# aipixel/GPS-Gaussian

Measured on NVIDIA H100. Metric: novel_views_per_sec_1024sq_500kgauss, higher is better.
Workload: dtype f32

## Files before the change

### gps-gaussian_b200/csrc/raster_render.cu

```cuda
#include "gpsg_internal.cuh"
#include "sm90_ptx.cuh"

namespace gpsg {

using namespace sm90;

struct f2p { float a, b; };
__device__ __forceinline__ f2p pk2(float lo, float hi) { return {lo, hi}; }
__device__ __forceinline__ void upk2(f2p v, float& lo, float& hi) { lo = v.a; hi = v.b; }
__device__ __forceinline__ f2p sub2(f2p x, f2p y) { return {__fsub_rn(x.a, y.a), __fsub_rn(x.b, y.b)}; }
__device__ __forceinline__ f2p mul2(f2p x, f2p y) { return {__fmul_rn(x.a, y.a), __fmul_rn(x.b, y.b)}; }
__device__ __forceinline__ f2p fma2(f2p x, f2p y, f2p z) { return {__fmaf_rn(x.a, y.a, z.a), __fmaf_rn(x.b, y.b, z.b)}; }

constexpr int kFwdWarps = 2;
constexpr int kFwdCTAsPerTile = 8 / kFwdWarps;
constexpr int kFwdQ = 32;
static_assert(kFwdWarps == 1 || kFwdWarps == 2 || kFwdWarps == 4, "a CTA holds 1, 2 or 4 of a tile's 8 blocks");

template <bool AUX>
struct FwdQueue {
    float4 A[2][kFwdQ], B[2][kFwdQ], C[2][kFwdQ];
    uint32_t pos[2][kFwdQ];
    float z[2][AUX ? kFwdQ : 1];
};

struct FwdPixel {
    float T = 1.0f, C0 = 0.0f, C1 = 0.0f, C2 = 0.0f, D = 0.0f;
    uint32_t last = 0;
    bool done;
};

template <bool AUX>
__device__ __forceinline__ void fwd_eval_pair(const float4& a0, const float4& a1, const float4& b0, const float4& b1,
                                              const float4& c0, const float4& c1, uint2 pos, float2 z, f2p pixfx2, f2p pixfy2,
                                              FwdPixel& px) {
    const f2p dx2 = sub2(pk2(a0.x, a1.x), pixfx2), dy2 = sub2(pk2(a0.y, a1.y), pixfy2);
    const f2p t2 = fma2(pk2(b0.x, b1.x), dx2, mul2(pk2(b0.y, b1.y), dy2));
    const f2p p2 = fma2(mul2(pk2(b0.z, b1.z), dy2), dy2, mul2(t2, dx2));
    float pA, pB;
    upk2(p2, pA, pB);
    float aA, aB;
    upk2(mul2(pk2(b0.w, b1.w), pk2(ex2_approx(pA), ex2_approx(pB))), aA, aB);
#pragma unroll
    for (int u = 0; u < 2; ++u) {
        const float p = u ? pB : pA;
        const float alpha = fminf(0.99f, u ? aB : aA);
        const bool valid = !px.done && !(p > 0.0f) && !(alpha < 1.0f / 255.0f);
        const float test_T = px.T * (1.0f - alpha);
        const bool stop = valid && (test_T < 0.0001f);
        const bool upd = valid && !stop;
        px.done = px.done || stop;
        const float w = upd ? alpha * px.T : 0.0f;
        const float4& c = u ? c1 : c0;
        px.C0 = fmaf(c.x, w, px.C0);
        px.C1 = fmaf(c.y, w, px.C1);
        px.C2 = fmaf(c.z, w, px.C2);
        if constexpr (AUX) px.D = fmaf(u ? z.y : z.x, w, px.D);
        px.T = upd ? test_T : px.T;
        px.last = upd ? (u ? pos.y : pos.x) : px.last;
    }
}

template <bool AUX>
__global__ void __launch_bounds__(kFwdWarps * 32, 32 / kFwdWarps) render_forward_kernel(const __grid_constant__ Camera cam,
                                                                            const float4* __restrict__ slabA,
                                                                            const float4* __restrict__ slabB,
                                                                            const float4* __restrict__ slabC,
                                                                            const uint32_t* __restrict__ blk_list,
                                                                            const uint2* __restrict__ ranges, const uint32_t* __restrict__ tile_order,
                                                                            const uint32_t* __restrict__ blk_count,
                                                                            const uint32_t* __restrict__ status,
                                                                            float* __restrict__ final_T,
                                                                            uint32_t* __restrict__ n_contrib,
                                                                            float* __restrict__ out_color,
                                                                            const float* __restrict__ depths,
                                                                            float* __restrict__ out_depth,
                                                                            float* __restrict__ out_alpha) {
    __shared__ FwdQueue<AUX> queues[kFwdWarps];
    const int lane = threadIdx.x & 31, warp = threadIdx.x >> 5;
    const int tile = (int)tile_order[blockIdx.x / kFwdCTAsPerTile];
    const int blk = (int)(blockIdx.x % kFwdCTAsPerTile) * kFwdWarps + warp;
    const int tile_y = tile / cam.grid_x, tile_x = tile - tile_y * cam.grid_x;
    int bx0, by0;
    fwd_block_origin(tile_x, tile_y, blk, bx0, by0);
    const int px = bx0 + (lane & 7), py = by0 + (lane >> 3);
    const bool inside = px < cam.W && py < cam.H;
    const uint2 range = status[2] ? make_uint2(0u, 0u) : ranges[tile];
    const uint32_t n = range.y - range.x;
    const int cnt = n ? (int)blk_count[8 * tile + blk] : 0;

    FwdPixel pix;
    pix.done = !inside;
    if (cnt > 0 && !__all_sync(0xffffffffu, pix.done)) {
        FwdQueue<AUX>& q = queues[warp];
        const uint32_t* __restrict__ list = blk_list + 8 * (size_t)range.x + (size_t)blk * n;
        const float4* __restrict__ tA = slabA + range.x;
        const float4* __restrict__ tB = slabB + range.x;
        const float4* __restrict__ tC = slabC + range.x;
        const f2p pixfx2 = pk2((float)px, (float)px), pixfy2 = pk2((float)py, (float)py);
        auto fetch = [&](int c, int buf, uint32_t p) {
            const int m = min(kFwdQ, cnt - c);
            if (lane < m) {
                cp_async16(&q.A[buf][lane], tA + p);
                cp_async16(&q.B[buf][lane], tB + p);
                cp_async16(&q.C[buf][lane], tC + p);
                q.pos[buf][lane] = p + 1u;
            } else if (lane == m && (m & 1)) {
                const float4 zero = make_float4(0.f, 0.f, 0.f, 0.f);
                q.A[buf][lane] = zero; q.B[buf][lane] = zero; q.C[buf][lane] = zero;
                q.pos[buf][lane] = 0u;
                if constexpr (AUX) q.z[buf][lane] = 0.f;
            }
        };
        auto fetch_z = [&](int c, int buf, uint32_t id) {
            if (lane < cnt - c) cp_async4(&q.z[buf][lane], depths + id);
        };
        uint32_t p = lane < cnt ? list[lane] : 0u;
        uint32_t id = 0u;
        fetch(0, 0, p);
        cp_async_commit();
        if constexpr (AUX) {
            if (lane < cnt) id = __float_as_uint(tC[p].w);
            fetch_z(0, 0, id);
            cp_async_commit();
        }
        p = lane + kFwdQ < cnt ? list[lane + kFwdQ] : 0u;
        for (int c = 0, buf = 0; c < cnt; c += kFwdQ, buf ^= 1) {
            const bool more = c + kFwdQ < cnt;
            if (more) {
                fetch(c + kFwdQ, buf ^ 1, p);
                if constexpr (AUX) { if (lane < cnt - c - kFwdQ) id = __float_as_uint(tC[p].w); }
                if (c + 2 * kFwdQ + lane < cnt) p = list[c + 2 * kFwdQ + lane];
            }
            cp_async_commit();
            cp_async_wait1();
            __syncwarp();
            const int m = min(kFwdQ, cnt - c);
#pragma unroll 2
            for (int i = 0; i < m; i += 2) {
                float2 z = make_float2(0.f, 0.f);
                if constexpr (AUX) z = *reinterpret_cast<const float2*>(&q.z[buf][i]);
                fwd_eval_pair<AUX>(q.A[buf][i], q.A[buf][i + 1], q.B[buf][i], q.B[buf][i + 1], q.C[buf][i], q.C[buf][i + 1],
                                   *reinterpret_cast<const uint2*>(&q.pos[buf][i]), z, pixfx2, pixfy2, pix);
            }
            __syncwarp();
            if (__all_sync(0xffffffffu, pix.done)) break;
            if constexpr (AUX) {
                if (more) fetch_z(c + kFwdQ, buf ^ 1, id);
                cp_async_commit();
            }
        }
        cp_async_wait_all();
    }

    if (inside) {
        const size_t HW = (size_t)cam.W * cam.H;
        const size_t pid = (size_t)py * cam.W + px;
        final_T[pid] = pix.T;
        n_contrib[pid] = pix.last;
        out_color[pid] = fmaf(pix.T, cam.bg[0], pix.C0);
        out_color[HW + pid] = fmaf(pix.T, cam.bg[1], pix.C1);
        out_color[2 * HW + pid] = fmaf(pix.T, cam.bg[2], pix.C2);
        if constexpr (AUX) {
            out_depth[pid] = pix.D;
            out_alpha[pid] = 1.0f - pix.T;
        }
    }
}

int launch_render_forward(const Camera& cam, BinningState b, ImageState im, float* out_color, const float* depths,
                          float* out_depth, float* out_alpha, cudaStream_t stream) {
    const unsigned grid = (unsigned)kFwdCTAsPerTile * (unsigned)(cam.grid_x * cam.grid_y);
    if (out_depth)
        render_forward_kernel<true><<<grid, kFwdWarps * 32, 0, stream>>>(
            cam, b.slabA, b.slabB, b.slabC, b.blk_list, im.ranges, im.tile_order, im.blk_count, im.totals, im.final_T,
            im.n_contrib, out_color, depths, out_depth, out_alpha);
    else
        render_forward_kernel<false><<<grid, kFwdWarps * 32, 0, stream>>>(
            cam, b.slabA, b.slabB, b.slabC, b.blk_list, im.ranges, im.tile_order, im.blk_count, im.totals, im.final_T,
            im.n_contrib, out_color, nullptr, nullptr, nullptr);
    GPSG_LAUNCH_CHECK();
    return GPSG_OK;
}

}
```

### gps-gaussian_b200/csrc/sm90_ptx.cuh

```cuda
#pragma once
#include <stdint.h>

namespace gpsg {
namespace sm90 {

__device__ __forceinline__ uint32_t smem_addr(const void* p) { return (uint32_t)__cvta_generic_to_shared(p); }

__device__ __forceinline__ float tf32(float x) {
    uint32_t r;
    asm("cvt.rna.tf32.f32 %0, %1;" : "=r"(r) : "f"(x));
    return __uint_as_float(r);
}

__device__ __forceinline__ float ex2_approx(float x) {
    float y;
    asm("ex2.approx.ftz.f32 %0, %1;" : "=f"(y) : "f"(x));
    return y;
}

__device__ __forceinline__ float rcp_approx(float x) {
    float y;
    asm("rcp.approx.ftz.f32 %0, %1;" : "=f"(y) : "f"(x));
    return y;
}

__device__ __forceinline__ uint32_t opaque(uint32_t x) {
    uint32_t y;
    asm volatile("mov.u32 %0, %1;" : "=r"(y) : "r"(x));
    return y;
}

__device__ __forceinline__ unsigned long long globaltimer() {
    unsigned long long t;
    asm volatile("mov.u64 %0, %%globaltimer;" : "=l"(t));
    return t;
}

__device__ __forceinline__ uint64_t gmma_desc(uint32_t addr, uint32_t lbo_bytes, uint32_t sbo_bytes) {
    uint64_t d = 0;
    d |= (uint64_t)((addr & 0x3FFFFu) >> 4);
    d |= (uint64_t)((lbo_bytes >> 4) & 0x3FFFu) << 16;
    d |= (uint64_t)((sbo_bytes >> 4) & 0x3FFFu) << 32;
    return d;
}

__device__ __forceinline__ void wgmma_m64n32k8(float (&d)[16], uint64_t a_desc, uint64_t b_desc) {
    asm volatile(
        "{\n\t.reg .pred p;\n\tsetp.ne.b32 p, %18, 0;\n\t"
        "wgmma.mma_async.sync.aligned.m64n32k8.f32.tf32.tf32 "
        "{%0, %1, %2, %3, %4, %5, %6, %7, %8, %9, %10, %11, %12, %13, %14, %15}, %16, %17, p, 1, 1;\n\t}"
        : "+f"(d[0]), "+f"(d[1]), "+f"(d[2]), "+f"(d[3]), "+f"(d[4]), "+f"(d[5]), "+f"(d[6]), "+f"(d[7]), "+f"(d[8]), "+f"(d[9]), "+f"(d[10]), "+f"(d[11]), "+f"(d[12]), "+f"(d[13]), "+f"(d[14]), "+f"(d[15])
        : "l"(a_desc), "l"(b_desc), "n"(1)
        : "memory");
}

__device__ __forceinline__ void wgmma_m64n48k8(float (&d)[24], uint64_t a_desc, uint64_t b_desc) {
    asm volatile(
        "{\n\t.reg .pred p;\n\tsetp.ne.b32 p, %26, 0;\n\t"
        "wgmma.mma_async.sync.aligned.m64n48k8.f32.tf32.tf32 "
        "{%0, %1, %2, %3, %4, %5, %6, %7, %8, %9, %10, %11, %12, %13, %14, %15, %16, %17, %18, %19, %20, %21, %22, %23}, %24, %25, p, 1, 1;\n\t}"
        : "+f"(d[0]), "+f"(d[1]), "+f"(d[2]), "+f"(d[3]), "+f"(d[4]), "+f"(d[5]), "+f"(d[6]), "+f"(d[7]), "+f"(d[8]), "+f"(d[9]), "+f"(d[10]), "+f"(d[11]), "+f"(d[12]), "+f"(d[13]), "+f"(d[14]), "+f"(d[15]), "+f"(d[16]), "+f"(d[17]), "+f"(d[18]), "+f"(d[19]), "+f"(d[20]), "+f"(d[21]), "+f"(d[22]), "+f"(d[23])
        : "l"(a_desc), "l"(b_desc), "n"(1)
        : "memory");
}

__device__ __forceinline__ void wgmma_m64n56k8(float (&d)[28], uint64_t a_desc, uint64_t b_desc) {
    asm volatile(
        "{\n\t.reg .pred p;\n\tsetp.ne.b32 p, %30, 0;\n\t"
        "wgmma.mma_async.sync.aligned.m64n56k8.f32.tf32.tf32 "
        "{%0, %1, %2, %3, %4, %5, %6, %7, %8, %9, %10, %11, %12, %13, %14, %15, %16, %17, %18, %19, %20, %21, %22, %23, %24, %25, %26, %27}, %28, %29, p, 1, 1;\n\t}"
        : "+f"(d[0]), "+f"(d[1]), "+f"(d[2]), "+f"(d[3]), "+f"(d[4]), "+f"(d[5]), "+f"(d[6]), "+f"(d[7]), "+f"(d[8]), "+f"(d[9]), "+f"(d[10]), "+f"(d[11]), "+f"(d[12]), "+f"(d[13]), "+f"(d[14]), "+f"(d[15]), "+f"(d[16]), "+f"(d[17]), "+f"(d[18]), "+f"(d[19]), "+f"(d[20]), "+f"(d[21]), "+f"(d[22]), "+f"(d[23]), "+f"(d[24]), "+f"(d[25]), "+f"(d[26]), "+f"(d[27])
        : "l"(a_desc), "l"(b_desc), "n"(1)
        : "memory");
}

__device__ __forceinline__ void wgmma_m64n64k8(float (&d)[32], uint64_t a_desc, uint64_t b_desc) {
    asm volatile(
        "{\n\t.reg .pred p;\n\tsetp.ne.b32 p, %34, 0;\n\t"
        "wgmma.mma_async.sync.aligned.m64n64k8.f32.tf32.tf32 "
        "{%0, %1, %2, %3, %4, %5, %6, %7, %8, %9, %10, %11, %12, %13, %14, %15, %16, %17, %18, %19, %20, %21, %22, %23, %24, %25, %26, %27, %28, %29, %30, %31}, %32, %33, p, 1, 1;\n\t}"
        : "+f"(d[0]), "+f"(d[1]), "+f"(d[2]), "+f"(d[3]), "+f"(d[4]), "+f"(d[5]), "+f"(d[6]), "+f"(d[7]), "+f"(d[8]), "+f"(d[9]), "+f"(d[10]), "+f"(d[11]), "+f"(d[12]), "+f"(d[13]), "+f"(d[14]), "+f"(d[15]), "+f"(d[16]), "+f"(d[17]), "+f"(d[18]), "+f"(d[19]), "+f"(d[20]), "+f"(d[21]), "+f"(d[22]), "+f"(d[23]), "+f"(d[24]), "+f"(d[25]), "+f"(d[26]), "+f"(d[27]), "+f"(d[28]), "+f"(d[29]), "+f"(d[30]), "+f"(d[31])
        : "l"(a_desc), "l"(b_desc), "n"(1)
        : "memory");
}

__device__ __forceinline__ void wgmma_m64n96k8(float (&d)[48], uint64_t a_desc, uint64_t b_desc) {
    asm volatile(
        "{\n\t.reg .pred p;\n\tsetp.ne.b32 p, %50, 0;\n\t"
        "wgmma.mma_async.sync.aligned.m64n96k8.f32.tf32.tf32 "
        "{%0, %1, %2, %3, %4, %5, %6, %7, %8, %9, %10, %11, %12, %13, %14, %15, %16, %17, %18, %19, %20, %21, %22, %23, %24, %25, %26, %27, %28, %29, %30, %31, %32, %33, %34, %35, %36, %37, %38, %39, %40, %41, %42, %43, %44, %45, %46, %47}, %48, %49, p, 1, 1;\n\t}"
        : "+f"(d[0]), "+f"(d[1]), "+f"(d[2]), "+f"(d[3]), "+f"(d[4]), "+f"(d[5]), "+f"(d[6]), "+f"(d[7]), "+f"(d[8]), "+f"(d[9]), "+f"(d[10]), "+f"(d[11]), "+f"(d[12]), "+f"(d[13]), "+f"(d[14]), "+f"(d[15]), "+f"(d[16]), "+f"(d[17]), "+f"(d[18]), "+f"(d[19]), "+f"(d[20]), "+f"(d[21]), "+f"(d[22]), "+f"(d[23]), "+f"(d[24]), "+f"(d[25]), "+f"(d[26]), "+f"(d[27]), "+f"(d[28]), "+f"(d[29]), "+f"(d[30]), "+f"(d[31]), "+f"(d[32]), "+f"(d[33]), "+f"(d[34]), "+f"(d[35]), "+f"(d[36]), "+f"(d[37]), "+f"(d[38]), "+f"(d[39]), "+f"(d[40]), "+f"(d[41]), "+f"(d[42]), "+f"(d[43]), "+f"(d[44]), "+f"(d[45]), "+f"(d[46]), "+f"(d[47])
        : "l"(a_desc), "l"(b_desc), "n"(1)
        : "memory");
}

template <int TA, int TB>
__device__ __forceinline__ void wgmma_m64n16k16_f16(float (&d)[8], uint64_t a_desc, uint64_t b_desc, int accumulate) {
    asm volatile(
        "{\n\t.reg .pred p;\n\t"
        "setp.ne.b32 p, %10, 0;\n\t"
        "wgmma.mma_async.sync.aligned.m64n16k16.f32.f16.f16 {%0, %1, %2, %3, %4, %5, %6, %7}, %8, %9, p, 1, 1, %11, %12;\n\t}"
        : "+f"(d[0]), "+f"(d[1]), "+f"(d[2]), "+f"(d[3]), "+f"(d[4]), "+f"(d[5]), "+f"(d[6]), "+f"(d[7])
        : "l"(a_desc), "l"(b_desc), "r"(accumulate), "n"(TA), "n"(TB)
        : "memory");
}

__device__ __forceinline__ void wgmma_m64n32k16_f16(float (&d)[16], uint64_t a_desc, uint64_t b_desc) {
    asm volatile(
        "{\n\t.reg .pred p;\n\tsetp.ne.b32 p, %18, 0;\n\t"
        "wgmma.mma_async.sync.aligned.m64n32k16.f32.f16.f16 "
        "{%0, %1, %2, %3, %4, %5, %6, %7, %8, %9, %10, %11, %12, %13, %14, %15}, %16, %17, p, 1, 1, 0, 0;\n\t}"
        : "+f"(d[0]), "+f"(d[1]), "+f"(d[2]), "+f"(d[3]), "+f"(d[4]), "+f"(d[5]), "+f"(d[6]), "+f"(d[7]), "+f"(d[8]), "+f"(d[9]), "+f"(d[10]), "+f"(d[11]), "+f"(d[12]), "+f"(d[13]), "+f"(d[14]), "+f"(d[15])
        : "l"(a_desc), "l"(b_desc), "n"(1)
        : "memory");
}

__device__ __forceinline__ void wgmma_m64n48k16_f16(float (&d)[24], uint64_t a_desc, uint64_t b_desc) {
    asm volatile(
        "{\n\t.reg .pred p;\n\tsetp.ne.b32 p, %26, 0;\n\t"
        "wgmma.mma_async.sync.aligned.m64n48k16.f32.f16.f16 "
        "{%0, %1, %2, %3, %4, %5, %6, %7, %8, %9, %10, %11, %12, %13, %14, %15, %16, %17, %18, %19, %20, %21, %22, %23}, %24, %25, p, 1, 1, 0, 0;\n\t}"
        : "+f"(d[0]), "+f"(d[1]), "+f"(d[2]), "+f"(d[3]), "+f"(d[4]), "+f"(d[5]), "+f"(d[6]), "+f"(d[7]), "+f"(d[8]), "+f"(d[9]), "+f"(d[10]), "+f"(d[11]), "+f"(d[12]), "+f"(d[13]), "+f"(d[14]), "+f"(d[15]), "+f"(d[16]), "+f"(d[17]), "+f"(d[18]), "+f"(d[19]), "+f"(d[20]), "+f"(d[21]), "+f"(d[22]), "+f"(d[23])
        : "l"(a_desc), "l"(b_desc), "n"(1)
        : "memory");
}

__device__ __forceinline__ void wgmma_m64n96k16_f16(float (&d)[48], uint64_t a_desc, uint64_t b_desc) {
    asm volatile(
        "{\n\t.reg .pred p;\n\tsetp.ne.b32 p, %50, 0;\n\t"
        "wgmma.mma_async.sync.aligned.m64n96k16.f32.f16.f16 "
        "{%0, %1, %2, %3, %4, %5, %6, %7, %8, %9, %10, %11, %12, %13, %14, %15, %16, %17, %18, %19, %20, %21, %22, %23, %24, %25, %26, %27, %28, %29, %30, %31, %32, %33, %34, %35, %36, %37, %38, %39, %40, %41, %42, %43, %44, %45, %46, %47}, %48, %49, p, 1, 1, 0, 0;\n\t}"
        : "+f"(d[0]), "+f"(d[1]), "+f"(d[2]), "+f"(d[3]), "+f"(d[4]), "+f"(d[5]), "+f"(d[6]), "+f"(d[7]), "+f"(d[8]), "+f"(d[9]), "+f"(d[10]), "+f"(d[11]), "+f"(d[12]), "+f"(d[13]), "+f"(d[14]), "+f"(d[15]), "+f"(d[16]), "+f"(d[17]), "+f"(d[18]), "+f"(d[19]), "+f"(d[20]), "+f"(d[21]), "+f"(d[22]), "+f"(d[23]), "+f"(d[24]), "+f"(d[25]), "+f"(d[26]), "+f"(d[27]), "+f"(d[28]), "+f"(d[29]), "+f"(d[30]), "+f"(d[31]), "+f"(d[32]), "+f"(d[33]), "+f"(d[34]), "+f"(d[35]), "+f"(d[36]), "+f"(d[37]), "+f"(d[38]), "+f"(d[39]), "+f"(d[40]), "+f"(d[41]), "+f"(d[42]), "+f"(d[43]), "+f"(d[44]), "+f"(d[45]), "+f"(d[46]), "+f"(d[47])
        : "l"(a_desc), "l"(b_desc), "n"(1)
        : "memory");
}

__device__ __forceinline__ void wgmma_m64n8k16_f16(float (&d)[4], uint64_t a_desc, uint64_t b_desc) {
    asm volatile(
        "{\n\t.reg .pred p;\n\tsetp.ne.b32 p, %6, 0;\n\t"
        "wgmma.mma_async.sync.aligned.m64n8k16.f32.f16.f16 "
        "{%0, %1, %2, %3}, %4, %5, p, 1, 1, 0, 0;\n\t}"
        : "+f"(d[0]), "+f"(d[1]), "+f"(d[2]), "+f"(d[3])
        : "l"(a_desc), "l"(b_desc), "n"(1)
        : "memory");
}
__device__ __forceinline__ void wgmma_m64n64k16_f16(float (&d)[32], uint64_t a_desc, uint64_t b_desc) {
    asm volatile(
        "{\n\t.reg .pred p;\n\tsetp.ne.b32 p, %34, 0;\n\t"
        "wgmma.mma_async.sync.aligned.m64n64k16.f32.f16.f16 "
        "{%0, %1, %2, %3, %4, %5, %6, %7, %8, %9, %10, %11, %12, %13, %14, %15, %16, %17, %18, %19, %20, %21, %22, %23, %24, %25, %26, %27, %28, %29, %30, %31}, %32, %33, p, 1, 1, 0, 0;\n\t}"
        : "+f"(d[0]), "+f"(d[1]), "+f"(d[2]), "+f"(d[3]), "+f"(d[4]), "+f"(d[5]), "+f"(d[6]), "+f"(d[7]), "+f"(d[8]), "+f"(d[9]), "+f"(d[10]), "+f"(d[11]), "+f"(d[12]), "+f"(d[13]), "+f"(d[14]), "+f"(d[15]), "+f"(d[16]), "+f"(d[17]), "+f"(d[18]), "+f"(d[19]), "+f"(d[20]), "+f"(d[21]), "+f"(d[22]), "+f"(d[23]), "+f"(d[24]), "+f"(d[25]), "+f"(d[26]), "+f"(d[27]), "+f"(d[28]), "+f"(d[29]), "+f"(d[30]), "+f"(d[31])
        : "l"(a_desc), "l"(b_desc), "n"(1)
        : "memory");
}
__device__ __forceinline__ void wgmma_m64n128k16_f16(float (&d)[64], uint64_t a_desc, uint64_t b_desc) {
    asm volatile(
        "{\n\t.reg .pred p;\n\tsetp.ne.b32 p, %66, 0;\n\t"
        "wgmma.mma_async.sync.aligned.m64n128k16.f32.f16.f16 "
        "{%0, %1, %2, %3, %4, %5, %6, %7, %8, %9, %10, %11, %12, %13, %14, %15, %16, %17, %18, %19, %20, %21, %22, %23, %24, %25, %26, %27, %28, %29, %30, %31, %32, %33, %34, %35, %36, %37, %38, %39, %40, %41, %42, %43, %44, %45, %46, %47, %48, %49, %50, %51, %52, %53, %54, %55, %56, %57, %58, %59, %60, %61, %62, %63}, %64, %65, p, 1, 1, 0, 0;\n\t}"
        : "+f"(d[0]), "+f"(d[1]), "+f"(d[2]), "+f"(d[3]), "+f"(d[4]), "+f"(d[5]), "+f"(d[6]), "+f"(d[7]), "+f"(d[8]), "+f"(d[9]), "+f"(d[10]), "+f"(d[11]), "+f"(d[12]), "+f"(d[13]), "+f"(d[14]), "+f"(d[15]), "+f"(d[16]), "+f"(d[17]), "+f"(d[18]), "+f"(d[19]), "+f"(d[20]), "+f"(d[21]), "+f"(d[22]), "+f"(d[23]), "+f"(d[24]), "+f"(d[25]), "+f"(d[26]), "+f"(d[27]), "+f"(d[28]), "+f"(d[29]), "+f"(d[30]), "+f"(d[31]), "+f"(d[32]), "+f"(d[33]), "+f"(d[34]), "+f"(d[35]), "+f"(d[36]), "+f"(d[37]), "+f"(d[38]), "+f"(d[39]), "+f"(d[40]), "+f"(d[41]), "+f"(d[42]), "+f"(d[43]), "+f"(d[44]), "+f"(d[45]), "+f"(d[46]), "+f"(d[47]), "+f"(d[48]), "+f"(d[49]), "+f"(d[50]), "+f"(d[51]), "+f"(d[52]), "+f"(d[53]), "+f"(d[54]), "+f"(d[55]), "+f"(d[56]), "+f"(d[57]), "+f"(d[58]), "+f"(d[59]), "+f"(d[60]), "+f"(d[61]), "+f"(d[62]), "+f"(d[63])
        : "l"(a_desc), "l"(b_desc), "n"(1)
        : "memory");
}
__device__ __forceinline__ void wgmma_m64n192k16_f16(float (&d)[96], uint64_t a_desc, uint64_t b_desc) {
    asm volatile(
        "{\n\t.reg .pred p;\n\tsetp.ne.b32 p, %98, 0;\n\t"
        "wgmma.mma_async.sync.aligned.m64n192k16.f32.f16.f16 "
        "{%0, %1, %2, %3, %4, %5, %6, %7, %8, %9, %10, %11, %12, %13, %14, %15, %16, %17, %18, %19, %20, %21, %22, %23, %24, %25, %26, %27, %28, %29, %30, %31, %32, %33, %34, %35, %36, %37, %38, %39, %40, %41, %42, %43, %44, %45, %46, %47, %48, %49, %50, %51, %52, %53, %54, %55, %56, %57, %58, %59, %60, %61, %62, %63, %64, %65, %66, %67, %68, %69, %70, %71, %72, %73, %74, %75, %76, %77, %78, %79, %80, %81, %82, %83, %84, %85, %86, %87, %88, %89, %90, %91, %92, %93, %94, %95}, %96, %97, p, 1, 1, 0, 0;\n\t}"
        : "+f"(d[0]), "+f"(d[1]), "+f"(d[2]), "+f"(d[3]), "+f"(d[4]), "+f"(d[5]), "+f"(d[6]), "+f"(d[7]), "+f"(d[8]), "+f"(d[9]), "+f"(d[10]), "+f"(d[11]), "+f"(d[12]), "+f"(d[13]), "+f"(d[14]), "+f"(d[15]), "+f"(d[16]), "+f"(d[17]), "+f"(d[18]), "+f"(d[19]), "+f"(d[20]), "+f"(d[21]), "+f"(d[22]), "+f"(d[23]), "+f"(d[24]), "+f"(d[25]), "+f"(d[26]), "+f"(d[27]), "+f"(d[28]), "+f"(d[29]), "+f"(d[30]), "+f"(d[31]), "+f"(d[32]), "+f"(d[33]), "+f"(d[34]), "+f"(d[35]), "+f"(d[36]), "+f"(d[37]), "+f"(d[38]), "+f"(d[39]), "+f"(d[40]), "+f"(d[41]), "+f"(d[42]), "+f"(d[43]), "+f"(d[44]), "+f"(d[45]), "+f"(d[46]), "+f"(d[47]), "+f"(d[48]), "+f"(d[49]), "+f"(d[50]), "+f"(d[51]), "+f"(d[52]), "+f"(d[53]), "+f"(d[54]), "+f"(d[55]), "+f"(d[56]), "+f"(d[57]), "+f"(d[58]), "+f"(d[59]), "+f"(d[60]), "+f"(d[61]), "+f"(d[62]), "+f"(d[63]), "+f"(d[64]), "+f"(d[65]), "+f"(d[66]), "+f"(d[67]), "+f"(d[68]), "+f"(d[69]), "+f"(d[70]), "+f"(d[71]), "+f"(d[72]), "+f"(d[73]), "+f"(d[74]), "+f"(d[75]), "+f"(d[76]), "+f"(d[77]), "+f"(d[78]), "+f"(d[79]), "+f"(d[80]), "+f"(d[81]), "+f"(d[82]), "+f"(d[83]), "+f"(d[84]), "+f"(d[85]), "+f"(d[86]), "+f"(d[87]), "+f"(d[88]), "+f"(d[89]), "+f"(d[90]), "+f"(d[91]), "+f"(d[92]), "+f"(d[93]), "+f"(d[94]), "+f"(d[95])
        : "l"(a_desc), "l"(b_desc), "n"(1)
        : "memory");
}
__device__ __forceinline__ void wgmma_m64n256k16_f16(float (&d)[128], uint64_t a_desc, uint64_t b_desc) {
    asm volatile(
        "{\n\t.reg .pred p;\n\tsetp.ne.b32 p, %130, 0;\n\t"
        "wgmma.mma_async.sync.aligned.m64n256k16.f32.f16.f16 "
        "{%0, %1, %2, %3, %4, %5, %6, %7, %8, %9, %10, %11, %12, %13, %14, %15, %16, %17, %18, %19, %20, %21, %22, %23, %24, %25, %26, %27, %28, %29, %30, %31, %32, %33, %34, %35, %36, %37, %38, %39, %40, %41, %42, %43, %44, %45, %46, %47, %48, %49, %50, %51, %52, %53, %54, %55, %56, %57, %58, %59, %60, %61, %62, %63, %64, %65, %66, %67, %68, %69, %70, %71, %72, %73, %74, %75, %76, %77, %78, %79, %80, %81, %82, %83, %84, %85, %86, %87, %88, %89, %90, %91, %92, %93, %94, %95, %96, %97, %98, %99, %100, %101, %102, %103, %104, %105, %106, %107, %108, %109, %110, %111, %112, %113, %114, %115, %116, %117, %118, %119, %120, %121, %122, %123, %124, %125, %126, %127}, %128, %129, p, 1, 1, 0, 0;\n\t}"
        : "+f"(d[0]), "+f"(d[1]), "+f"(d[2]), "+f"(d[3]), "+f"(d[4]), "+f"(d[5]), "+f"(d[6]), "+f"(d[7]), "+f"(d[8]), "+f"(d[9]), "+f"(d[10]), "+f"(d[11]), "+f"(d[12]), "+f"(d[13]), "+f"(d[14]), "+f"(d[15]), "+f"(d[16]), "+f"(d[17]), "+f"(d[18]), "+f"(d[19]), "+f"(d[20]), "+f"(d[21]), "+f"(d[22]), "+f"(d[23]), "+f"(d[24]), "+f"(d[25]), "+f"(d[26]), "+f"(d[27]), "+f"(d[28]), "+f"(d[29]), "+f"(d[30]), "+f"(d[31]), "+f"(d[32]), "+f"(d[33]), "+f"(d[34]), "+f"(d[35]), "+f"(d[36]), "+f"(d[37]), "+f"(d[38]), "+f"(d[39]), "+f"(d[40]), "+f"(d[41]), "+f"(d[42]), "+f"(d[43]), "+f"(d[44]), "+f"(d[45]), "+f"(d[46]), "+f"(d[47]), "+f"(d[48]), "+f"(d[49]), "+f"(d[50]), "+f"(d[51]), "+f"(d[52]), "+f"(d[53]), "+f"(d[54]), "+f"(d[55]), "+f"(d[56]), "+f"(d[57]), "+f"(d[58]), "+f"(d[59]), "+f"(d[60]), "+f"(d[61]), "+f"(d[62]), "+f"(d[63]), "+f"(d[64]), "+f"(d[65]), "+f"(d[66]), "+f"(d[67]), "+f"(d[68]), "+f"(d[69]), "+f"(d[70]), "+f"(d[71]), "+f"(d[72]), "+f"(d[73]), "+f"(d[74]), "+f"(d[75]), "+f"(d[76]), "+f"(d[77]), "+f"(d[78]), "+f"(d[79]), "+f"(d[80]), "+f"(d[81]), "+f"(d[82]), "+f"(d[83]), "+f"(d[84]), "+f"(d[85]), "+f"(d[86]), "+f"(d[87]), "+f"(d[88]), "+f"(d[89]), "+f"(d[90]), "+f"(d[91]), "+f"(d[92]), "+f"(d[93]), "+f"(d[94]), "+f"(d[95]), "+f"(d[96]), "+f"(d[97]), "+f"(d[98]), "+f"(d[99]), "+f"(d[100]), "+f"(d[101]), "+f"(d[102]), "+f"(d[103]), "+f"(d[104]), "+f"(d[105]), "+f"(d[106]), "+f"(d[107]), "+f"(d[108]), "+f"(d[109]), "+f"(d[110]), "+f"(d[111]), "+f"(d[112]), "+f"(d[113]), "+f"(d[114]), "+f"(d[115]), "+f"(d[116]), "+f"(d[117]), "+f"(d[118]), "+f"(d[119]), "+f"(d[120]), "+f"(d[121]), "+f"(d[122]), "+f"(d[123]), "+f"(d[124]), "+f"(d[125]), "+f"(d[126]), "+f"(d[127])
        : "l"(a_desc), "l"(b_desc), "n"(1)
        : "memory");
}

template <int N>
__device__ __forceinline__ void fence_acc(float (&acc)[N]) {
#pragma unroll
    for (int i = 0; i < N; ++i) asm volatile("" : "+f"(acc[i])::"memory");
}
template <int NC>
__device__ __forceinline__ void fence_acc(float (&acc)[NC][8]) {
#pragma unroll
    for (int c = 0; c < NC; ++c) fence_acc(acc[c]);
}

__device__ __forceinline__ void wgmma_fence() { asm volatile("wgmma.fence.sync.aligned;" ::: "memory"); }
__device__ __forceinline__ void wgmma_commit() { asm volatile("wgmma.commit_group.sync.aligned;" ::: "memory"); }
__device__ __forceinline__ void wgmma_wait() { asm volatile("wgmma.wait_group.sync.aligned 0;" ::: "memory"); }
__device__ __forceinline__ void fence_async() { asm volatile("fence.proxy.async.shared::cta;" ::: "memory"); }

__device__ __forceinline__ void mma_m16n8k8(float (&d)[4], const float (&a)[4], float b0, float b1) {
    asm volatile("mma.sync.aligned.m16n8k8.row.col.f32.tf32.tf32.f32 {%0, %1, %2, %3}, {%4, %5, %6, %7}, {%8, %9}, "
                 "{%0, %1, %2, %3};"
                 : "+f"(d[0]), "+f"(d[1]), "+f"(d[2]), "+f"(d[3])
                 : "r"(__float_as_uint(a[0])), "r"(__float_as_uint(a[1])), "r"(__float_as_uint(a[2])),
                   "r"(__float_as_uint(a[3])), "r"(__float_as_uint(b0)), "r"(__float_as_uint(b1)));
}

__device__ __forceinline__ void cp_async16(void* smem, const void* gmem) {
    asm volatile("cp.async.cg.shared.global [%0], [%1], 16;" ::"r"(smem_addr(smem)), "l"(gmem) : "memory");
}
__device__ __forceinline__ void cp_async16_zfill(void* smem, const void* gmem, uint32_t src_bytes) {
    asm volatile("cp.async.cg.shared.global [%0], [%1], 16, %2;" ::"r"(smem_addr(smem)), "l"(gmem), "r"(src_bytes)
                 : "memory");
}
__device__ __forceinline__ void cp_async4(void* smem, const void* gmem) {
    asm volatile("cp.async.ca.shared.global [%0], [%1], 4;" ::"r"(smem_addr(smem)), "l"(gmem) : "memory");
}
__device__ __forceinline__ void cp_async_commit() { asm volatile("cp.async.commit_group;" ::: "memory"); }
__device__ __forceinline__ void cp_async_wait1() { asm volatile("cp.async.wait_group 1;" ::: "memory"); }
__device__ __forceinline__ void cp_async_wait_all() { asm volatile("cp.async.wait_all;" ::: "memory"); }

}
}
```

Measured before the change: 5672.

## Render two horizontally adjacent pixels per thread with half-warp quarter-tile queues

Each thread now shades two adjacent pixels, and each half-warp handles one of a tile's four quarter-tile blocks with its own Gaussian queue. Per-Gaussian shared loads and the dy-dependent products are reused across both pixels, and only the xy part of slab A is fetched (8-byte cp.async). The done flag is folded into the sign of T, and outputs are written as float2 stores when the width is even. The trade-off is twice the per-thread accumulator state, and both half-warps now loop to the larger of their two counts. The code also relies on blk_count and fwd_block_origin meaning quarter-tile blocks even though the indexing still uses 8*tile, so it depends on how binning was set up.

```diff
diff --git a/gps-gaussian_b200/csrc/raster_render.cu b/gps-gaussian_b200/csrc/raster_render.cu
--- a/gps-gaussian_b200/csrc/raster_render.cu
+++ b/gps-gaussian_b200/csrc/raster_render.cu
@@ -5,60 +5,50 @@
 
 using namespace sm90;
 
-struct f2p { float a, b; };
-__device__ __forceinline__ f2p pk2(float lo, float hi) { return {lo, hi}; }
-__device__ __forceinline__ void upk2(f2p v, float& lo, float& hi) { lo = v.a; hi = v.b; }
-__device__ __forceinline__ f2p sub2(f2p x, f2p y) { return {__fsub_rn(x.a, y.a), __fsub_rn(x.b, y.b)}; }
-__device__ __forceinline__ f2p mul2(f2p x, f2p y) { return {__fmul_rn(x.a, y.a), __fmul_rn(x.b, y.b)}; }
-__device__ __forceinline__ f2p fma2(f2p x, f2p y, f2p z) { return {__fmaf_rn(x.a, y.a, z.a), __fmaf_rn(x.b, y.b, z.b)}; }
-
 constexpr int kFwdWarps = 2;
-constexpr int kFwdCTAsPerTile = 8 / kFwdWarps;
+constexpr int kFwdCTAsPerTile = 4 / kFwdWarps;
 constexpr int kFwdQ = 32;
-static_assert(kFwdWarps == 1 || kFwdWarps == 2 || kFwdWarps == 4, "a CTA holds 1, 2 or 4 of a tile's 8 blocks");
+static_assert(kFwdWarps == 1 || kFwdWarps == 2, "a CTA holds 1 or 2 of a tile's 4 quarter tiles");
 
 template <bool AUX>
 struct FwdQueue {
-    float4 A[2][kFwdQ], B[2][kFwdQ], C[2][kFwdQ];
-    uint32_t pos[2][kFwdQ];
-    float z[2][AUX ? kFwdQ : 1];
+    float2 A[2][kFwdQ][2];
+    float4 B[2][kFwdQ][2], C[2][kFwdQ][2];
+    uint2 pos[2][kFwdQ / 2][2];
+    float2 z[2][AUX ? kFwdQ / 2 : 1][2];
 };
 
 struct FwdPixel {
     float T = 1.0f, C0 = 0.0f, C1 = 0.0f, C2 = 0.0f, D = 0.0f;
     uint32_t last = 0;
-    bool done;
 };
 
 template <bool AUX>
-__device__ __forceinline__ void fwd_eval_pair(const float4& a0, const float4& a1, const float4& b0, const float4& b1,
-                                              const float4& c0, const float4& c1, uint2 pos, float2 z, f2p pixfx2, f2p pixfy2,
-                                              FwdPixel& px) {
-    const f2p dx2 = sub2(pk2(a0.x, a1.x), pixfx2), dy2 = sub2(pk2(a0.y, a1.y), pixfy2);
-    const f2p t2 = fma2(pk2(b0.x, b1.x), dx2, mul2(pk2(b0.y, b1.y), dy2));
-    const f2p p2 = fma2(mul2(pk2(b0.z, b1.z), dy2), dy2, mul2(t2, dx2));
-    float pA, pB;
-    upk2(p2, pA, pB);
-    float aA, aB;
-    upk2(mul2(pk2(b0.w, b1.w), pk2(ex2_approx(pA), ex2_approx(pB))), aA, aB);
-#pragma unroll
-    for (int u = 0; u < 2; ++u) {
-        const float p = u ? pB : pA;
-        const float alpha = fminf(0.99f, u ? aB : aA);
-        const bool valid = !px.done && !(p > 0.0f) && !(alpha < 1.0f / 255.0f);
-        const float test_T = px.T * (1.0f - alpha);
-        const bool stop = valid && (test_T < 0.0001f);
-        const bool upd = valid && !stop;
-        px.done = px.done || stop;
-        const float w = upd ? alpha * px.T : 0.0f;
-        const float4& c = u ? c1 : c0;
-        px.C0 = fmaf(c.x, w, px.C0);
-        px.C1 = fmaf(c.y, w, px.C1);
-        px.C2 = fmaf(c.z, w, px.C2);
-        if constexpr (AUX) px.D = fmaf(u ? z.y : z.x, w, px.D);
-        px.T = upd ? test_T : px.T;
-        px.last = upd ? (u ? pos.y : pos.x) : px.last;
-    }
+__device__ __forceinline__ void fwd_blend(float p, float alpha, const float4& c, uint32_t pos, float z, FwdPixel& px) {
+    const bool skip = p > 0.0f || alpha < 1.0f / 255.0f;
+    const float test_T = px.T * (1.0f - alpha);
+    const bool upd = !skip && !(test_T < 0.0001f);
+    const float w = upd ? alpha * px.T : 0.0f;
+    px.C0 = fmaf(c.x, w, px.C0);
+    px.C1 = fmaf(c.y, w, px.C1);
+    px.C2 = fmaf(c.z, w, px.C2);
+    if constexpr (AUX) px.D = fmaf(z, w, px.D);
+    px.T = upd ? test_T : (skip ? px.T : -fabsf(px.T));
+    px.last = upd ? pos : px.last;
+}
+
+template <bool AUX>
+__device__ __forceinline__ void fwd_eval(const float2& a, const float4& b, const float4& c, uint32_t pos, float z, float fx0,
+                                         float fx1, float fy, FwdPixel& px0, FwdPixel& px1) {
+    const float dy = __fsub_rn(a.y, fy);
+    const float bydy = __fmul_rn(b.y, dy), bzdy = __fmul_rn(b.z, dy);
+    const float dx0 = __fsub_rn(a.x, fx0), dx1 = __fsub_rn(a.x, fx1);
+    const float p0 = __fmaf_rn(bzdy, dy, __fmul_rn(__fmaf_rn(b.x, dx0, bydy), dx0));
+    const float p1 = __fmaf_rn(bzdy, dy, __fmul_rn(__fmaf_rn(b.x, dx1, bydy), dx1));
+    const float al0 = fminf(0.99f, __fmul_rn(b.w, ex2_approx(p0)));
+    const float al1 = fminf(0.99f, __fmul_rn(b.w, ex2_approx(p1)));
+    fwd_blend<AUX>(p0, al0, c, pos, z, px0);
+    fwd_blend<AUX>(p1, al1, c, pos, z, px1);
 }
 
 template <bool AUX>
@@ -78,92 +68,129 @@
                                                                             float* __restrict__ out_alpha) {
     __shared__ FwdQueue<AUX> queues[kFwdWarps];
     const int lane = threadIdx.x & 31, warp = threadIdx.x >> 5;
+    const int half = lane >> 4, hl = lane & 15;
     const int tile = (int)tile_order[blockIdx.x / kFwdCTAsPerTile];
-    const int blk = (int)(blockIdx.x % kFwdCTAsPerTile) * kFwdWarps + warp;
+    const int blk = 2 * ((int)(blockIdx.x % kFwdCTAsPerTile) * kFwdWarps + warp) + half;
     const int tile_y = tile / cam.grid_x, tile_x = tile - tile_y * cam.grid_x;
     int bx0, by0;
     fwd_block_origin(tile_x, tile_y, blk, bx0, by0);
-    const int px = bx0 + (lane & 7), py = by0 + (lane >> 3);
-    const bool inside = px < cam.W && py < cam.H;
+    const int px = bx0 + 2 * (hl & 3), py = by0 + (hl >> 2);
+    const bool in0 = px < cam.W && py < cam.H, in1 = px + 1 < cam.W && py < cam.H;
     const uint2 range = status[2] ? make_uint2(0u, 0u) : ranges[tile];
     const uint32_t n = range.y - range.x;
     const int cnt = n ? (int)blk_count[8 * tile + blk] : 0;
-
-    FwdPixel pix;
-    pix.done = !inside;
-    if (cnt > 0 && !__all_sync(0xffffffffu, pix.done)) {
+    const int cnt_max = max(cnt, __shfl_xor_sync(0xffffffffu, cnt, 16));
+
+    FwdPixel pix0, pix1;
+    pix0.T = in0 ? 1.0f : -1.0f;
+    pix1.T = in1 ? 1.0f : -1.0f;
+    if (cnt_max > 0 && !__all_sync(0xffffffffu, cnt == 0 || (pix0.T < 0.0f && pix1.T < 0.0f))) {
         FwdQueue<AUX>& q = queues[warp];
         const uint32_t* __restrict__ list = blk_list + 8 * (size_t)range.x + (size_t)blk * n;
         const float4* __restrict__ tA = slabA + range.x;
         const float4* __restrict__ tB = slabB + range.x;
         const float4* __restrict__ tC = slabC + range.x;
-        const f2p pixfx2 = pk2((float)px, (float)px), pixfy2 = pk2((float)py, (float)py);
-        auto fetch = [&](int c, int buf, uint32_t p) {
-            const int m = min(kFwdQ, cnt - c);
-            if (lane < m) {
-                cp_async16(&q.A[buf][lane], tA + p);
-                cp_async16(&q.B[buf][lane], tB + p);
-                cp_async16(&q.C[buf][lane], tC + p);
-                q.pos[buf][lane] = p + 1u;
-            } else if (lane == m && (m & 1)) {
+        const float fx0 = (float)px, fx1 = (float)(px + 1), fy = (float)py;
+        auto put = [&](int c, int buf, int s, uint32_t p) {
+            uint32_t& ps = reinterpret_cast<uint32_t*>(&q.pos[buf][s >> 1][half])[s & 1];
+            if (c + s < cnt) {
+                cp_async8(&q.A[buf][s][half], tA + p);
+                cp_async16(&q.B[buf][s][half], tB + p);
+                cp_async16(&q.C[buf][s][half], tC + p);
+                ps = p + 1u;
+            } else {
                 const float4 zero = make_float4(0.f, 0.f, 0.f, 0.f);
-                q.A[buf][lane] = zero; q.B[buf][lane] = zero; q.C[buf][lane] = zero;
-                q.pos[buf][lane] = 0u;
-                if constexpr (AUX) q.z[buf][lane] = 0.f;
+                q.A[buf][s][half] = make_float2(0.f, 0.f); q.B[buf][s][half] = zero; q.C[buf][s][half] = zero;
+                ps = 0u;
+                if constexpr (AUX) reinterpret_cast<float*>(&q.z[buf][s >> 1][half])[s & 1] = 0.f;
             }
         };
-        auto fetch_z = [&](int c, int buf, uint32_t id) {
-            if (lane < cnt - c) cp_async4(&q.z[buf][lane], depths + id);
+        auto fetch = [&](int c, int buf, uint32_t p0, uint32_t p1) {
+            put(c, buf, hl, p0);
+            put(c, buf, hl + 16, p1);
         };
-        uint32_t p = lane < cnt ? list[lane] : 0u;
-        uint32_t id = 0u;
-        fetch(0, 0, p);
+        auto fetch_z = [&](int c, int buf, uint32_t id0, uint32_t id1) {
+            if (c + hl < cnt) cp_async4(reinterpret_cast<float*>(&q.z[buf][hl >> 1][half]) + (hl & 1), depths + id0);
+            if (c + hl + 16 < cnt)
+                cp_async4(reinterpret_cast<float*>(&q.z[buf][(hl + 16) >> 1][half]) + (hl & 1), depths + id1);
+        };
+        auto list_at = [&](int i) { return i < cnt ? list[i] : 0u; };
+        uint32_t p0 = list_at(hl), p1 = list_at(hl + 16);
+        uint32_t id0 = 0u, id1 = 0u;
+        fetch(0, 0, p0, p1);
         cp_async_commit();
         if constexpr (AUX) {
-            if (lane < cnt) id = __float_as_uint(tC[p].w);
-            fetch_z(0, 0, id);
+            if (hl < cnt) id0 = __float_as_uint(tC[p0].w);
+            if (hl + 16 < cnt) id1 = __float_as_uint(tC[p1].w);
+            fetch_z(0, 0, id0, id1);
             cp_async_commit();
         }
-        p = lane + kFwdQ < cnt ? list[lane + kFwdQ] : 0u;
-        for (int c = 0, buf = 0; c < cnt; c += kFwdQ, buf ^= 1) {
-            const bool more = c + kFwdQ < cnt;
+        p0 = list_at(kFwdQ + hl);
+        p1 = list_at(kFwdQ + hl + 16);
+        for (int c = 0, buf = 0; c < cnt_max; c += kFwdQ, buf ^= 1) {
+            const bool more = c + kFwdQ < cnt_max;
             if (more) {
-                fetch(c + kFwdQ, buf ^ 1, p);
-                if constexpr (AUX) { if (lane < cnt - c - kFwdQ) id = __float_as_uint(tC[p].w); }
-                if (c + 2 * kFwdQ + lane < cnt) p = list[c + 2 * kFwdQ + lane];
+                fetch(c + kFwdQ, buf ^ 1, p0, p1);
+                if constexpr (AUX) {
+                    if (c + kFwdQ + hl < cnt) id0 = __float_as_uint(tC[p0].w);
+                    if (c + kFwdQ + hl + 16 < cnt) id1 = __float_as_uint(tC[p1].w);
+                }
+                p0 = list_at(c + 2 * kFwdQ + hl);
+                p1 = list_at(c + 2 * kFwdQ + hl + 16);
             }
             cp_async_commit();
             cp_async_wait1();
             __syncwarp();
-            const int m = min(kFwdQ, cnt - c);
+            const int m = min(kFwdQ, cnt_max - c);
 #pragma unroll 2
             for (int i = 0; i < m; i += 2) {
+                const uint2 pos = q.pos[buf][i >> 1][half];
                 float2 z = make_float2(0.f, 0.f);
-                if constexpr (AUX) z = *reinterpret_cast<const float2*>(&q.z[buf][i]);
-                fwd_eval_pair<AUX>(q.A[buf][i], q.A[buf][i + 1], q.B[buf][i], q.B[buf][i + 1], q.C[buf][i], q.C[buf][i + 1],
-                                   *reinterpret_cast<const uint2*>(&q.pos[buf][i]), z, pixfx2, pixfy2, pix);
+                if constexpr (AUX) z = q.z[buf][i >> 1][half];
+                fwd_eval<AUX>(q.A[buf][i][half], q.B[buf][i][half], q.C[buf][i][half], pos.x, z.x, fx0, fx1, fy, pix0, pix1);
+                fwd_eval<AUX>(q.A[buf][i + 1][half], q.B[buf][i + 1][half], q.C[buf][i + 1][half], pos.y, z.y, fx0, fx1, fy,
+                              pix0, pix1);
             }
             __syncwarp();
-            if (__all_sync(0xffffffffu, pix.done)) break;
+            if (__all_sync(0xffffffffu, c + kFwdQ >= cnt || (pix0.T < 0.0f && pix1.T < 0.0f))) break;
             if constexpr (AUX) {
-                if (more) fetch_z(c + kFwdQ, buf ^ 1, id);
+                if (more) fetch_z(c + kFwdQ, buf ^ 1, id0, id1);
                 cp_async_commit();
             }
         }
         cp_async_wait_all();
     }
 
-    if (inside) {
-        const size_t HW = (size_t)cam.W * cam.H;
-        const size_t pid = (size_t)py * cam.W + px;
-        final_T[pid] = pix.T;
-        n_contrib[pid] = pix.last;
-        out_color[pid] = fmaf(pix.T, cam.bg[0], pix.C0);
-        out_color[HW + pid] = fmaf(pix.T, cam.bg[1], pix.C1);
-        out_color[2 * HW + pid] = fmaf(pix.T, cam.bg[2], pix.C2);
+    const size_t HW = (size_t)cam.W * cam.H;
+    const size_t pid = (size_t)py * cam.W + px;
+    const float T0 = fabsf(pix0.T), T1 = fabsf(pix1.T);
+    if (!(cam.W & 1)) {
+        if (!in0) return;
+        auto st2 = [&](float* base, float v0, float v1) { *reinterpret_cast<float2*>(base + pid) = make_float2(v0, v1); };
+        st2(final_T, T0, T1);
+        *reinterpret_cast<uint2*>(n_contrib + pid) = make_uint2(pix0.last, pix1.last);
+        st2(out_color, fmaf(T0, cam.bg[0], pix0.C0), fmaf(T1, cam.bg[0], pix1.C0));
+        st2(out_color + HW, fmaf(T0, cam.bg[1], pix0.C1), fmaf(T1, cam.bg[1], pix1.C1));
+        st2(out_color + 2 * HW, fmaf(T0, cam.bg[2], pix0.C2), fmaf(T1, cam.bg[2], pix1.C2));
         if constexpr (AUX) {
-            out_depth[pid] = pix.D;
-            out_alpha[pid] = 1.0f - pix.T;
+            st2(out_depth, pix0.D, pix1.D);
+            st2(out_alpha, 1.0f - T0, 1.0f - T1);
+        }
+        return;
+    }
+#pragma unroll
+    for (int u = 0; u < 2; ++u) {
+        const FwdPixel& pix = u ? pix1 : pix0;
+        if (!(u ? in1 : in0)) continue;
+        const float T = fabsf(pix.T);
+        final_T[pid + u] = T;
+        n_contrib[pid + u] = pix.last;
+        out_color[pid + u] = fmaf(T, cam.bg[0], pix.C0);
+        out_color[HW + pid + u] = fmaf(T, cam.bg[1], pix.C1);
+        out_color[2 * HW + pid + u] = fmaf(T, cam.bg[2], pix.C2);
+        if constexpr (AUX) {
+            out_depth[pid + u] = pix.D;
+            out_alpha[pid + u] = 1.0f - T;
         }
     }
 }
diff --git a/gps-gaussian_b200/csrc/sm90_ptx.cuh b/gps-gaussian_b200/csrc/sm90_ptx.cuh
--- a/gps-gaussian_b200/csrc/sm90_ptx.cuh
+++ b/gps-gaussian_b200/csrc/sm90_ptx.cuh
@@ -212,6 +212,9 @@
     asm volatile("cp.async.cg.shared.global [%0], [%1], 16, %2;" ::"r"(smem_addr(smem)), "l"(gmem), "r"(src_bytes)
                  : "memory");
 }
+__device__ __forceinline__ void cp_async8(void* smem, const void* gmem) {
+    asm volatile("cp.async.ca.shared.global [%0], [%1], 8;" ::"r"(smem_addr(smem)), "l"(gmem) : "memory");
+}
 __device__ __forceinline__ void cp_async4(void* smem, const void* gmem) {
     asm volatile("cp.async.ca.shared.global [%0], [%1], 4;" ::"r"(smem_addr(smem)), "l"(gmem) : "memory");
 }
```

Result: faster. 5829 (median of 6 runs) (+2.8%).
